# alphafox02/iridium-sniffer

Hardware: AMD Instinct MI355X
Metric: IQ Msamples/s end-to-end (detect->demod), 10 MHz cf32 (higher is better)
Workload: dtype f32

## Files before the change

iridium-sniffer_amd/csrc/scan_band.hip:

```cpp
#include <atomic>
#include <mutex>
#include "common.hpp"
#include "types.hpp"
#include "kernels.hpp"
#include "band_core.hpp"
#include "band_wave.hpp"

namespace irdm {

namespace {

__device__ __forceinline__ bool band_void(const BandParams &P, const BandWork &W)
{
    return __hip_atomic_load(W.bar + 5, __ATOMIC_RELAXED, __HIP_MEMORY_SCOPE_AGENT) == (unsigned)P.serial;
}

struct TlScope {
    unsigned long long *lo, *hi;
    __device__ __forceinline__ TlScope(const BandParams &P, const BandWork &W, int slot) : lo(nullptr), hi(nullptr)
    {
        if (P.tl_sel >= 0 && (threadIdx.x & 63) == 0 && slot >= 0 && slot < kBandTlSlots) {
            lo = W.tl + (size_t)P.tl_sel * 2 * kBandTlSlots + slot;
            hi = lo + kBandTlSlots;
            atomicMin(lo, (unsigned long long)wall_clock64());
// ... 49 lines not shown
    int bad = 0, ca = 0, cb = 0;
    for (int a = lane; a < na; a += 64) {
        if (A[a].cb < X - P.hw || A[a].cb >= X + P.hw) continue;
        ca++;
        bool found = false;
        for (int b = 0; b < nb && !found; b++) found = B[b].cb == A[a].cb && band_rec_same(A[a], B[b]);
        if (!found) bad = 1;
    }
    for (int b = lane; b < nb; b += 64)
        if (B[b].cb >= X - P.hw && B[b].cb < X + P.hw) cb++;
    for (int d = 32; d; d >>= 1) {
        ca += __shfl_xor(ca, d);
        cb += __shfl_xor(cb, d);
        bad |= __shfl_xor(bad, d);
    }
    return !(bad || ca != cb);
}

struct ZoneEnt {
    uint32_t cb, start_lo, idx;
};
constexpr int kZoneCap = 32;
constexpr size_t kZoneLdsBytes = 64 * kZoneCap * (sizeof(ZoneEnt) + sizeof(uint32_t)) + 128 * sizeof(uint32_t);

__device__ void boundaries_agree_lds(const BandParams &P, const BandWork &W, uint8_t *lds, int *s_fail, int nt)
{
    ZoneEnt *zb = reinterpret_cast<ZoneEnt *>(lds);
    uint32_t *za = reinterpret_cast<uint32_t *>(zb + 64 * kZoneCap);
    uint32_t *zc = za + 64 * kZoneCap;
    const int tid = threadIdx.x, gl = tid & 15;
    for (int t = tid; t < 128; t += nt) zc[t] = 0;
    __syncthreads();
    for (int i = tid >> 4; i + 1 < P.n_bands; i += nt >> 4) {
        const int X = (i + 1) * P.band_w;
        const BandRec *A = W.recs + (size_t)i * kBandRecCap, *B = W.recs + (size_t)(i + 1) * kBandRecCap;
        const int na = min((int)W.rec_count[i], kBandRecCap), nb = min((int)W.rec_count[i + 1], kBandRecCap);
        const int nmax = max(na, nb);
        for (int k = gl; k < nmax; k += 16) {
            const int cba = k < na ? A[k].cb : -0x40000000;
            const int cbb = k < nb ? B[k].cb : -0x40000000;
            const uint32_t stb = k < nb ? (uint32_t)B[k].start : 0u;
            if (cba >= X - P.hw && cba < X + P.hw) {
                const uint32_t at = atomicAdd(&zc[2 * i], 1u);
                if (at < (uint32_t)kZoneCap) za[i * kZoneCap + at] = (uint32_t)k;
            }
            if (cbb >= X - P.hw && cbb < X + P.hw) {
                const uint32_t at = atomicAdd(&zc[2 * i + 1], 1u);
                if (at < (uint32_t)kZoneCap) zb[i * kZoneCap + at] = ZoneEnt{ (uint32_t)cbb, stb, (uint32_t)k };
            }
        }
    }
    __syncthreads();
    int bad = 0;
    for (int i = tid >> 4; i + 1 < P.n_bands; i += nt >> 4) {
        const int X = (i + 1) * P.band_w;
        const BandRec *A = W.recs + (size_t)i * kBandRecCap, *B = W.recs + (size_t)(i + 1) * kBandRecCap;
        const int na = min((int)W.rec_count[i], kBandRecCap), nb = min((int)W.rec_count[i + 1], kBandRecCap);
        const int ca = (int)zc[2 * i], cb = (int)zc[2 * i + 1];
        if (ca != cb) {
            bad = 1;
        } else if (ca > kZoneCap) {
            for (int a = gl; a < na; a += 16) {
                if (A[a].cb < X - P.hw || A[a].cb >= X + P.hw) continue;
                bool found = false;
                for (int b = 0; b < nb && !found; b++) found = B[b].cb == A[a].cb && band_rec_same(A[a], B[b]);
                if (!found) bad = 1;
            }
        } else {
            for (int k = gl; k < ca; k += 16) {
                const BandRec ra = A[za[i * kZoneCap + k]];
                bool found = false;
                for (int j = 0; j < cb && !found; j++) {
                    const ZoneEnt e = zb[i * kZoneCap + j];
                    if (e.cb == (uint32_t)ra.cb && e.start_lo == (uint32_t)ra.start) found = band_rec_same(ra, B[e.idx]);
                }
                if (!found) bad = 1;
            }
        }
    }
    if (bad) atomicOr(s_fail, 1);
}

__device__ __forceinline__ SumStep make_step(const BandParams &P, int uf, int old, int slot)
{
    SumStep s;
    const uint32_t row = (uint32_t)P.n * 4u;
    s.nw_off = (uint32_t)uf * row;
    s.ol_off = (uint32_t)(old < 0 ? -old - 1 : old) * row;
    s.snap_off = slot >= 0 ? (uint32_t)slot * row : ~0u;
    s.pad = 0;
    return s;
}
__device__ __forceinline__ SumStep noop_step()
{
    SumStep s;
    s.nw_off = 0;
    s.ol_off = 0;
    s.snap_off = ~0u;
    s.pad = 0;
    return s;
}

struct PlanShared {
    int32_t part[kPlanThreads / 64 + 1];
    int mismatch, first, status, agree_fail;
    unsigned flags;
    int kstar;
};

constexpr int kPlanLdsFrames = 8192;
constexpr size_t kPlanLdsBytes = ((2 * kPlanLdsFrames + 2 + 15) & ~15) + sizeof(int32_t) * (2 * kPlanLdsFrames + 2);
static_assert(kZoneLdsBytes <= kPlanLdsBytes, "the boundary test's lists live in the plan's LDS before the plan needs it");

template <int NT>
__device__ void band_plan_body(const BandParams &P, const BandWork &W, const unsigned *__restrict__ counts,
                               DetState *__restrict__ st, int round, PlanShared &sh, uint8_t *lds,
                               const uint64_t *u_busy = nullptr, const uint64_t *u_forced = nullptr)
{
    const bool first = round == 0 || (P.spec_in && round == 1);
    if (!(P.spec_in && round == 1) || u_busy == nullptr) {
        u_busy = W.busy;
        u_forced = W.forced;
    }
    constexpr int kPlanThreads = NT;
    int32_t *s_part = sh.part;
    int &s_mismatch = sh.mismatch, &s_first = sh.first, &s_status = sh.status, &s_agree_fail = sh.agree_fail;
    unsigned &s_flags = sh.flags;
    const int tid = threadIdx.x;
    BandCtl *ctl = W.ctl;
    if (first) {
        if (tid == 0) {
            const unsigned prev = W.bar[4];
            s_status = (P.chained && prev != 1u) ? 1 : 0;
            if (s_status) __hip_atomic_store(W.bar + 5, (unsigned)P.serial, __ATOMIC_RELAXED, __HIP_MEMORY_SCOPE_AGENT);
            else W.bar[4] = 0;
        }
        __syncthreads();
        if (s_status) return;
        __syncthreads();
    } else if (band_void(P, W)) {
        return;
    }
    if (first) {
        if (tid < (int)(sizeof(BandCtl) / 4)) reinterpret_cast<uint32_t *>(ctl)[tid] = 0;
        if (tid == 0) {
            *W.flags = 0;
            st->n_gone = 0;
        }
        __syncthreads();
        if (round != 0 && tid == 0) ctl->h0 = st->hist_idx;
    }
    if (ctl->status != 0) return;
    const int F = P.n_frames;
    const uint64_t t_begin = wall_clock64();
    uint32_t *tp = ctl->tp + (round == 1 ? 0 : 8);
    auto stamp = [&](int i) {
        if (tid == 0 && round >= 1) tp[i] = (uint32_t)(wall_clock64() - t_begin);
    };

    if (tid == 0) {
        s_mismatch = 0;
        s_first = 0x7fffffff;
        s_flags = 0;
        s_status = 0;
        s_agree_fail = 0;
    }
    __syncthreads();
    if (round == 0) {
        int any = 0;
        for (int f = tid; f < F; f += kPlanThreads) {
            const unsigned c = counts[f];
            W.uq[f] = 0;
            W.uf[f] = 0;
            W.cnt_before[f] = 0;
            const int slot = c > 0 ? 0 : -1;
            W.slot_pre[f] = slot;
            W.slot_post[f] = slot;
            any |= c > 0 ? 1 : 0;
            if (c > (unsigned)P.list_cap) atomicOr(&s_flags, BAND_F_LIST);
        }
        if (any) atomicOr(&s_mismatch, 1);
        for (int i = tid; i < P.n_bands * P.occ_words; i += kPlanThreads) W.occ[i] = 0;
        for (int i = tid; i < P.occ_words; i += kPlanThreads) {
            W.busy[i] = 0;
            W.forced[i] = 0;
            W.conc[i] = 0;
        }
        for (int i = tid; i < P.n_bands; i += kPlanThreads) W.rec_count[i] = 0;
        for (int k = tid; k < 2 * kSumDepth + 1; k += kPlanThreads) W.steps[k] = noop_step();
        __syncthreads();
        if (tid == 0) {
            const int some = s_mismatch;
            ctl->h0 = st->hist_idx;
            W.need[0] = some;
            W.snap_slot[0] = some ? 0 : -1;
            ctl->n_upd = 0;
            ctl->n_snap = some;
            ctl->rounds = 1;
            if (s_flags) {
                ctl->flags = s_flags;
                ctl->status = 2;
            }
        }
        return;
    } else if (first) {
        for (int f = tid; f < F; f += kPlanThreads)
            if (counts[f] > (unsigned)P.list_cap) atomicOr(&s_flags, BAND_F_LIST);
        __syncthreads();
        if (s_flags) {
            if (tid == 0) {
                ctl->flags = s_flags;
                ctl->rounds = 1;
                ctl->status = 2;
            }
            return;
        }
        for (int f = tid; f < F; f += kPlanThreads) {
            W.uq[f] = ((u_busy[f >> 6] >> (f & 63)) & 1) ? 0 : 1;
            W.uf[f] = (uint8_t)((u_forced[f >> 6] >> (f & 63)) & 1);
        }
        if (P.selfcheck & 32) {
            __syncthreads();
            if (tid == 0 && F >= 8) W.uq[(3 * F) / 4] ^= 1;
            __syncthreads();
        }
    } else {
        for (int f = tid; f < F; f += kPlanThreads) {
            const int q = ((W.busy[f >> 6] >> (f & 63)) & 1) ? 0 : 1;
            const int fc = (int)((W.forced[f >> 6] >> (f & 63)) & 1);
            if (q != W.uq[f] || fc != W.uf[f]) {
                atomicAdd(&s_mismatch, 1);
                atomicMin(&s_first, f);
            }
        }
        for (int b = tid; b < P.occ_words; b += kPlanThreads)
            if (W.conc[b] >= (unsigned)P.max_bursts) atomicOr(&s_flags, BAND_F_SQUELCH);
        __syncthreads();
        stamp(0);
        if (P.selfcheck & 2) {
            for (int i = 1; i < P.n_bands; i++) {
                BandRec *B = W.recs + (size_t)i * kBandRecCap;
                const int X = i * P.band_w, nb = min((int)W.rec_count[i], kBandRecCap);
                for (int k = tid; k < nb; k += kPlanThreads)
                    if (B[k].cb >= X - P.hw && B[k].cb < X + P.hw) B[k].last_active += 1;
            }
            __syncthreads();
        }
        if (lds != nullptr) {
            boundaries_agree_lds(P, W, lds, &s_agree_fail, NT);
            if (P.selfcheck & 1) {
                __shared__ int s_other;
                if (tid == 0) s_other = 0;
                __syncthreads();
                for (int i = tid >> 6; i + 1 < P.n_bands; i += kPlanThreads / 64)
                    if (!boundary_agrees(P, W, i, tid & 63) && (tid & 63) == 0) atomicOr(&s_other, 1);
                __syncthreads();
                if (tid == 0 && s_other != s_agree_fail) atomicOr(&s_flags, BAND_F_CHECK);
            }
        } else {
            for (int i = tid >> 6; i + 1 < P.n_bands; i += kPlanThreads / 64)
                if (!boundary_agrees(P, W, i, tid & 63) && (tid & 63) == 0) atomicOr(&s_agree_fail, 1);
        }
        __syncthreads();
        stamp(1);
        if (tid == 0) {
            unsigned fl = s_flags | *W.flags;
            int status = 0;
            if (fl) {
                status = 2;
            } else if (s_mismatch == 0) {
                if (s_agree_fail) {
                    fl |= BAND_F_AGREE;
                    status = 2;
                } else {
                    status = 1;
                }
            } else if (round >= kBandRounds) {
                fl |= BAND_F_ITER;
                status = 2;
            }
            ctl->flags = fl;
            ctl->mismatch = s_mismatch;
            ctl->first_mismatch = s_first;
            ctl->rounds = round;
            ctl->status = status;
            s_status = status;
        }
        __syncthreads();
        if (s_status != 0) return;
        for (int f = tid; f < F; f += kPlanThreads) {
            W.uq[f] = ((W.busy[f >> 6] >> (f & 63)) & 1) ? 0 : 1;
            W.uf[f] = (uint8_t)((W.forced[f >> 6] >> (f & 63)) & 1);
        }
    }
    __syncthreads();
    if (round == 0 && s_flags) {
        if (tid == 0) {
            ctl->flags = s_flags;
            ctl->status = 2;
        }
        return;
    }

    if (lds != nullptr && F <= kPlanLdsFrames) {
        constexpr int FPT = kPlanLdsFrames / NT;
        uint8_t *s_need = lds;
        int32_t *s_slot = reinterpret_cast<int32_t *>(lds + ((2 * kPlanLdsFrames + 2 + 15) & ~15));
        const int f0 = tid * FPT;
        int uqb = 0, ufb = 0, cnz = 0, c_t = 0;
#pragma unroll
        for (int j = 0; j < FPT; j++) {
            const int f = f0 + j;
            if (f < F) {
                int q = ((u_busy[f >> 6] >> (f & 63)) & 1) ? 0 : 1;
                const int fc = (int)((u_forced[f >> 6] >> (f & 63)) & 1);
                if ((P.selfcheck & 32) && first && round == 1 && F >= 8 && f == (3 * F) / 4) q ^= 1;
                uqb |= q << j;
                ufb |= fc << j;
                cnz |= (counts[f] > 0 ? 1 : 0) << j;
                c_t += q + fc;
            }
        }
        __syncthreads();
        stamp(2);
        for (int i = tid; i < P.n_bands * P.occ_words; i += kPlanThreads) W.occ[i] = 0;
        for (int i = tid; i < P.occ_words; i += kPlanThreads) {
            W.busy[i] = 0;
            W.forced[i] = 0;
            W.conc[i] = 0;
        }
        for (int i = tid; i < P.n_bands; i += kPlanThreads) W.rec_count[i] = 0;
        const int lane = tid & 63, wave = tid >> 6;
        auto scan1 = [&](int v, int &total) {
            int incl = v;
            for (int d = 1; d < 64; d <<= 1) {
                const int o = __shfl_up(incl, d);
                if (lane >= d) incl += o;
            }
            if (lane == 63) s_part[wave] = incl;
            __syncthreads();
            int wb = 0, tot = 0;
            for (int w = 0; w < NT / 64; w++) {
                const int o = s_part[w];
                if (w < wave) wb += o;
                tot += o;
            }
            __syncthreads();
            total = tot;
            return wb + incl - v;
        };
        int n_upd = 0;
        const int base = scan1(c_t, n_upd);
        stamp(3);
        for (int k = tid; k <= n_upd + 1; k += kPlanThreads) s_need[k] = (P.sum_restart && k > 0 && (k & 63) == 0) ? 1 : 0;
        __syncthreads();
        {
            int k = base;
#pragma unroll
            for (int j = 0; j < FPT; j++) {
                const int f = f0 + j;
                if (f < F) {
                    const int q = (uqb >> j) & 1, fc = (ufb >> j) & 1;
                    if (f == s_first) sh.kstar = k;
                    if ((cnz >> j) & 1) {
                        s_need[k] = 1;
                        if (fc) s_need[k + 1] = 1;
                    }
                    if (fc) W.upd_frame[k++] = f;
                    if (q) W.upd_frame[k++] = f;
                }
            }
        }
        __syncthreads();
        stamp(4);
        const int kpt = (n_upd + 1 + NT - 1) / NT;
        const int k0 = tid * kpt, k1 = min(k0 + kpt, n_upd + 1);
        int nn = 0;
        for (int k = k0; k < k1; k++) nn += s_need[k];
        int n_snap = 0;
        int run = scan1(nn, n_snap);
        for (int k = k0; k < k1; k++) {
            const int nd = s_need[k];
            s_slot[k] = nd ? run : -1;
            run += nd;
        }
        if (tid == 0) W.snap_slot[0] = s_need[0] ? 0 : -1;
        __syncthreads();
        stamp(5);
        const int h0 = ctl->h0;
        for (int k = n_upd + tid; k < n_upd + 2 * kSumDepth + 1; k += kPlanThreads) W.steps[k] = noop_step();
        for (int k = tid; k < n_upd; k += kPlanThreads) {
            const int uf_k = W.upd_frame[k];
            const int old = k < kHistory ? -(((h0 + k) % kHistory) + 1) : W.upd_frame[k - kHistory];
            W.steps[k] = make_step(P, uf_k, old, s_slot[k + 1]);
        }
        {
            int k = base;
#pragma unroll
            for (int j = 0; j < FPT; j++) {
                const int f = f0 + j;
                if (f < F) {
                    const int q = (uqb >> j) & 1, fc = (ufb >> j) & 1, has = (cnz >> j) & 1;
                    const int pre = has ? s_slot[k] : -1;
                    W.slot_pre[f] = pre;
                    W.slot_post[f] = (has && fc) ? s_slot[k + 1] : pre;
                    k += q + fc;
                }
            }
        }
        __syncthreads();
        stamp(6);
        if (tid == 0) {
            ctl->n_upd = n_upd;
            ctl->n_snap = n_snap;
            ctl->rounds = round + 1;
            if (n_snap > W.snap_cap) {
                ctl->flags = BAND_F_SNAP;
                ctl->status = 2;
            }
            int kr = 0;
            if (P.sum_restart && !first && round >= 2 && s_first != 0x7fffffff && s_first < F) kr = (sh.kstar / 64) * 64;
            if (kr > n_upd) kr = (n_upd / 64) * 64;
            if (kr >= 64 && s_slot[kr] >= 0) {
                ctl->k_restart = kr;
                ctl->restart_slot = s_slot[kr];
                ctl->n_restarts++;
            } else {
                ctl->k_restart = 0;
                ctl->restart_slot = -1;
            }
        }
        return;
    }

    for (int i = tid; i < P.n_bands * P.occ_words; i += kPlanThreads) W.occ[i] = 0;
    for (int i = tid; i < P.occ_words; i += kPlanThreads) {
        W.busy[i] = 0;
        W.forced[i] = 0;
        W.conc[i] = 0;
    }
    for (int i = tid; i < P.n_bands; i += kPlanThreads) W.rec_count[i] = 0;

    for (int f = tid; f < F; f += kPlanThreads) W.tmp[f] = W.uq[f] + W.uf[f];
    __syncthreads();
    const int n_upd = block_scan<NT>(W.tmp, W.cnt_before, F, s_part);
    for (int k = tid; k <= n_upd; k += kPlanThreads) W.need[k] = 0;
    __syncthreads();
    for (int f = tid; f < F; f += kPlanThreads) {
        int k = W.cnt_before[f];
        if (counts[f] > 0) {
            W.need[k] = 1;
            if (W.uf[f]) W.need[k + 1] = 1;
        }
        if (W.uf[f]) W.upd_frame[k++] = f;
        if (W.uq[f]) W.upd_frame[k] = f;
    }
    __syncthreads();
    const int n_snap = block_scan<NT>(W.need, W.tmp, n_upd + 1, s_part);
    for (int k = tid; k <= n_upd; k += kPlanThreads) W.snap_slot[k] = W.need[k] ? W.tmp[k] : -1;
    __syncthreads();
    const int h0 = ctl->h0;
    for (int k = n_upd + tid; k < n_upd + 2 * kSumDepth + 1; k += kPlanThreads) W.steps[k] = noop_step();
    for (int k = tid; k < n_upd; k += kPlanThreads) {
        W.snap_after[k] = W.snap_slot[k + 1];
        W.old_row[k] = k < kHistory ? -(((h0 + k) % kHistory) + 1) : W.upd_frame[k - kHistory];
        W.steps[k] = make_step(P, W.upd_frame[k], W.old_row[k], W.snap_after[k]);
    }
    for (int f = tid; f < F; f += kPlanThreads) {
        const int k = W.cnt_before[f];
        const int pre = counts[f] > 0 ? W.snap_slot[k] : -1;
        W.slot_pre[f] = pre;
        W.slot_post[f] = (counts[f] > 0 && W.uf[f]) ? W.snap_slot[k + 1] : pre;
    }
    if (tid == 0) {
        ctl->n_upd = n_upd;
        ctl->n_snap = n_snap;
// ... 110 lines not shown
        const bool more = k0 + 2 * kSumDepth < n;
        const uint4 dnn = steps4[k0 + 4 * kSumDepth + lane];
        IRDM_SUM_LOAD(nwB, olB, d, 1, k0 + kSumDepth)
        IRDM_SUM_CONSUME(nwA, olA, d, 0, k0)
        if (more) { IRDM_SUM_LOAD(nwA, olA, dn, 0, k0 + 2 * kSumDepth) }
        IRDM_SUM_CONSUME(nwB, olB, d, 1, k0 + kSumDepth)
        d = dn;
        dn = dnn;
    }
#undef IRDM_SUM_LOAD
#undef IRDM_SUM_CONSUME
#undef IRDM_SUM_STEP
    W.sum_new[b] = s;
    smin_out[b] = smin;
    if (!(pre[b] <= 0.9f * P.thr * smin)) atomicOr(W.flags, BAND_F_STALE);
}

__global__ __launch_bounds__(64) void band_sum_kernel(BandParams P, BandWork W, const float *__restrict__ mag,
                                                      const float *__restrict__ hist, const float *__restrict__ sum,
                                                      const float *__restrict__ pre, float *__restrict__ smin_out,
                                                      const SumStep *__restrict__ steps, float *__restrict__ snap)
{
    IRDM_DETECTOR_PRIO();
    TlScope tl(P, W, 4 * (W.ctl->rounds - 1) + 1);
    if (band_void(P, W) || W.ctl->status != 0) return;
    band_sum_body(P, W, mag, hist, sum, pre, smin_out, steps, snap, (int)blockIdx.x * 64 + (int)threadIdx.x);
}

constexpr int kWalkWaveGroups = 256;

template <int NW>
__global__ __launch_bounds__(256) void band_walk_wave_kernel(BandParams P, BandWork W, BandIO io, const DetState *__restrict__ st)
{
    IRDM_DETECTOR_PRIO();
    TlScope tl(P, W, 4 * (W.ctl->rounds - 1) + 3);
    if (band_void(P, W) || W.ctl->status != 0) return;
    io.act_in = st->act;
    io.n_act_in = (int32_t)wv_first((uint32_t)st->n_act);
    const int lane = threadIdx.x & 63;
    const int gw = (int)wv_first((uint32_t)(blockIdx.x * 4 + (threadIdx.x >> 6))), n_waves = (int)gridDim.x * 4;
    const int n_pairs = P.n_bands * P.occ_words;
    unsigned long long *tl_stat = nullptr;
    if (P.tl_sel >= 0)
        tl_stat = W.tl + (size_t)P.tl_sel * 2 * kBandTlSlots + kBandTlSlots + (W.ctl->rounds - 1 == 0 ? 26 : 28);
    int wave_events = 0;
    const unsigned long long t_wave = tl_stat ? wall_clock64() : 0;
    for (int p0 = gw; p0 < n_pairs; p0 += 64 * n_waves) {
        const int pl = p0 + lane * n_waves;
        bool work = false;
        if (pl < n_pairs) {
            const int band = pl / P.occ_words, blk = pl % P.occ_words;
            work = blk == 0 || band_segment_starts(io.occ + (size_t)band * P.occ_words, blk, P.gap, false) != 0;
        }
        uint64_t todo = __builtin_amdgcn_ballot_w64(work);
        while (todo) {
            const int j = __builtin_ctzll(todo);
            todo &= todo - 1;
            const int p = p0 + j * n_waves;
            const int band = p / P.occ_words, blk = p % P.occ_words;
            bool carried = false;
            int events = 0;
            if (blk == 0) {
                WaveWalker<NW> w(P, io, band, lane);
                if (w.load_carried() > 0) {
                    carried = true;
                    w.run(0, true);
                    events += w.n_events;
                }
            }
            uint64_t starts = wv_first64(band_segment_starts(io.occ + (size_t)band * P.occ_words, blk, P.gap, carried));
            while (starts) {
                const int q = __builtin_ctzll(starts);
                starts &= starts - 1;
                WaveWalker<NW> w(P, io, band, lane);
                w.run(64 * blk + q, false);
                events += w.n_events;
            }
            wave_events += events;
            if (tl_stat && lane == 0) {
                atomicMax(tl_stat, (unsigned long long)events);
                atomicAdd(tl_stat + 1, (unsigned long long)events);
            }
        }
    }
    if (tl_stat && lane == 0 && W.ctl->rounds - 1 != 0) {
        unsigned long long *x = W.tl + (size_t)P.tl_sel * 2 * kBandTlSlots + kBandTlSlots + 30;
        atomicMax(x, (unsigned long long)wave_events);
        atomicMax(x + 1, wall_clock64() - t_wave);
    }
}

__device__ __forceinline__ void band_cross_wave(const BandParams &P, const BandWork &W, unsigned c,
                                                const ListEntry *__restrict__ entries, int f, uint32_t *s_bits, int lane)
{
    const int N = P.n;
    for (int w = lane; w < N / 32; w += 64) s_bits[w] = 0;
    __builtin_amdgcn_fence(__ATOMIC_RELEASE, "wavefront");
    __builtin_amdgcn_wave_barrier();
    const float *srow = W.snap + (size_t)W.slot_pre[f] * N;
    const ListEntry *e = entries + (size_t)f * P.list_cap;
    float *rq = W.relq + (size_t)f * N;
    for (unsigned i = lane; i < c; i += 64) {
        const int bin = e[i].bin;
        const float base = srow[bin];
        const float rel = base > 0 ? e[i].mag / base : 0.0f;
        if (rel > P.thr) {
            atomicOr(&s_bits[bin >> 5], 1u << (bin & 31));
            rq[bin] = rel;
        }
    }
    __builtin_amdgcn_fence(__ATOMIC_ACQ_REL, "wavefront");
    __builtin_amdgcn_wave_barrier();
    uint32_t *out = reinterpret_cast<uint32_t *>(W.cross) + (size_t)f * (N / 32);
    for (int w = lane; w < N / 32; w += 64) out[w] = s_bits[w];
    if (lane < P.n_bands) {
        const int w0 = (lane * P.band_w - P.band_w / 2) / 32, nw = 2 * P.band_w / 32;
        uint32_t any = 0;
        for (int k = 0; k < nw; k++) {
            const int w = w0 + k;
            if (w >= 0 && w < N / 32) any |= s_bits[w];
        }
        if (any) atomicOr(reinterpret_cast<unsigned long long *>(&W.occ[(size_t)lane * P.occ_words + (f >> 6)]), 1ull << (f & 63));
    }
    __builtin_amdgcn_fence(__ATOMIC_ACQ_REL, "wavefront");
    __builtin_amdgcn_wave_barrier();
}

constexpr int kCrossGroups = 256;

__global__ __launch_bounds__(256) void band_cross_w_kernel(BandParams P, BandWork W, const unsigned *__restrict__ counts,
                                                           const ListEntry *__restrict__ entries)
{
    IRDM_DETECTOR_PRIO();
    TlScope tl(P, W, 4 * (W.ctl->rounds - 1) + 2);
    __shared__ uint32_t s_bits_all[4][16384 / 32];
    if (band_void(P, W) || W.ctl->status != 0) return;
    const int lane = threadIdx.x & 63, wave = threadIdx.x >> 6;
    const int gw = (int)blockIdx.x * 4 + wave, n_waves = (int)gridDim.x * 4;
    uint32_t *s_bits = s_bits_all[wave];
    for (int f0 = gw; f0 < P.n_frames; f0 += 64 * n_waves) {
        const int fl = f0 + lane * n_waves;
        const unsigned cl = fl < P.n_frames ? counts[fl] : 0u;
        uint64_t todo = __builtin_amdgcn_ballot_w64(cl != 0 && cl <= (unsigned)P.list_cap);
        while (todo) {
            const int j = __builtin_ctzll(todo);
            todo &= todo - 1;
            const unsigned c = (unsigned)__builtin_amdgcn_readlane((int)cl, j);
            band_cross_wave(P, W, c, entries, f0 + j * n_waves, s_bits, lane);
        }
    }
}


__global__ __launch_bounds__(256) void band_spec_prep_kernel(BandParams P, BandWork S, const unsigned *__restrict__ counts,
                                                              const float *__restrict__ sum_src, DetState *__restrict__ st_spec,
                                                              int have_prev)
{
    IRDM_DETECTOR_PRIO();
    const int tid = threadIdx.x, F = P.n_frames;
    __shared__ unsigned s_n;
    if (tid == 0) s_n = 0;
    __syncthreads();
    if (have_prev)
        for (int band = tid >> 4; band < P.n_bands; band += 256 / 16) {
            const int cnt = min((int)S.rec_count[band], kBandRecCap);
            for (int j = tid & 15; j < cnt; j += 16) {
                const BandRec &r = S.recs[(size_t)band * kBandRecCap + j];
                if (!(r.flags & 1) || r.stop >= 0) continue;
                const unsigned at = atomicAdd(&s_n, 1u);
                if (at < (unsigned)kMaxActive) {
                    ActiveBurst a;
                    a.id = 0; a.start = (uint64_t)r.start; a.last_active = (uint64_t)r.last_active;
                    a.center_bin = r.cb; a.peak_rel = r.rel; a.base_sum = r.base; a.pad = 0;
                    st_spec->act[at] = a;
                }
            }
        }
    __syncthreads();
    if (tid == 0) st_spec->n_act = (uint32_t)min(s_n, (unsigned)kMaxActive);
    if (tid < (int)(sizeof(BandCtl) / 4)) reinterpret_cast<uint32_t *>(S.ctl)[tid] = 0;
    for (int f = tid; f < F; f += 256) {
        const int slot = counts[f] > 0 ? 0 : -1;
        S.slot_pre[f] = slot;
        S.slot_post[f] = slot;
    }
    for (int i = tid; i < P.n_bands * P.occ_words; i += 256) S.occ[i] = 0;
    for (int i = tid; i < P.occ_words; i += 256) {
        S.busy[i] = 0;
        S.forced[i] = 0;
        S.conc[i] = 0;
    }
    for (int i = tid; i < P.n_bands; i += 256) S.rec_count[i] = 0;
    for (int b = tid; b < P.n; b += 256) S.snap[b] = sum_src[b];
    __syncthreads();
    if (tid == 0) {
        *S.flags = 0;
        S.ctl->rounds = 1;
        S.snap_slot[0] = 0;
    }
}

__device__ void lds_bitonic_sort(uint64_t *key, uint16_t *val, int np)
{
    for (int k = 2; k <= np; k <<= 1) {
        for (int j = k >> 1; j > 0; j >>= 1) {
            for (int i = threadIdx.x; i < np / 2; i += blockDim.x) {
                const int lo = ((i & ~(j - 1)) << 1) | (i & (j - 1)), hi = lo | j;
                const uint64_t a = key[lo], b = key[hi];
                if ((a > b) == ((lo & k) == 0)) {
                    key[lo] = b;
                    key[hi] = a;
                    const uint16_t va = val[lo];
                    val[lo] = val[hi];
                    val[hi] = va;
                }
            }
            __syncthreads();
        }
    }
}

__device__ void band_commit_body(const BandParams &P, const BandWork &W, DetState *__restrict__ st,
                                 float *__restrict__ sum, GoneBurst *__restrict__ gone, int gone_cap,
                                 unsigned char *smem_raw)
{
    const int kPlanThreads = (int)blockDim.x;
    uint64_t *s_key = reinterpret_cast<uint64_t *>(smem_raw);
    uint16_t *s_val = reinterpret_cast<uint16_t *>(s_key + kBandMaxTotal);
    uint32_t *rank_of = W.rank;
    __shared__ unsigned s_n, s_carried, s_gone;
    BandCtl *ctl = W.ctl;
    if (band_void(P, W) || ctl->status != 1 || ctl->committed) return;
    const int tid = threadIdx.x;
    if (tid == 0) {
        s_n = 0;
        s_carried = 0;
        s_gone = 0;
    }
    __syncthreads();
    for (int band = tid >> 4; band < P.n_bands; band += kPlanThreads / 16) {
        {
            const int cnt = min((int)W.rec_count[band], kBandRecCap);
            for (int j = tid & 15; j < cnt; j += 16) {
                const int i = band * kBandRecCap + j;
                const BandRec &r = W.recs[i];
                if (!(r.flags & 1)) continue;
                const unsigned at = atomicAdd(&s_n, 1u);
                if (at < (unsigned)kBandMaxTotal) W.tot[at] = i;
                if (r.cf < 0) atomicAdd(&s_carried, 1u);
                if (r.stop >= 0) atomicAdd(&s_gone, 1u);
            }
        }
    }
    __syncthreads();
    const int n = (int)s_n, n_carried = (int)s_carried, n_gone = (int)s_gone;
    if (n > kBandMaxTotal || n_gone > gone_cap) {
        if (tid == 0) {
            ctl->flags |= n > kBandMaxTotal ? BAND_F_TOTAL : BAND_F_GONECAP;
            ctl->n_gone = n_gone;
            ctl->status = 2;
        }
        return;
    }
    for (int t = tid; t < n; t += kPlanThreads) {
        const BandRec &r = W.recs[W.tot[t]];
        uint64_t key;
        if (r.cf < 0) {
            key = (uint64_t)r.seq;
        } else {
            uint32_t rb;
            __builtin_memcpy(&rb, &r.rel, 4);
            key = (1ull << 63) | ((uint64_t)r.cf << 46) | ((uint64_t)(0xffffffffu - rb) << 14) | (uint64_t)r.cb;
        }
        s_key[t] = key;
        s_val[t] = (uint16_t)t;
    }
    int np = 2;
    while (np < n) np <<= 1;
    for (int t = n + tid; t < np; t += kPlanThreads) {
        s_key[t] = ~0ull;
        s_val[t] = 0xffff;
    }
    __syncthreads();
    lds_bitonic_sort(s_key, s_val, np);
    for (int q = tid; q < n; q += kPlanThreads) rank_of[s_val[q]] = (uint32_t)q;
    __syncthreads();
    const uint64_t id0 = st->burst_id;
    for (int t = tid; t < n; t += kPlanThreads) {
        const BandRec &r = W.recs[W.tot[t]];
        W.ids[t] = r.cf < 0 ? st->act[r.seq].id : id0 + 10ull * (uint64_t)((int)rank_of[t] - n_carried);
    }
    for (int t = tid; t < n; t += kPlanThreads) {
        const BandRec &r = W.recs[W.tot[t]];
        s_key[t] = r.stop >= 0 ? (((uint64_t)((r.stop - (int64_t)P.idx0) >> P.log_n)) << 32) | rank_of[t]
                               : (1ull << 63) | rank_of[t];
        s_val[t] = (uint16_t)t;
    }
    for (int t = n + tid; t < np; t += kPlanThreads) {
        s_key[t] = ~0ull;
        s_val[t] = 0xffff;
    }
    __syncthreads();
    lds_bitonic_sort(s_key, s_val, np);
    for (int pos = tid; pos < n; pos += kPlanThreads) {
        const int t = s_val[pos];
        const BandRec &r = W.recs[W.tot[t]];
        const uint64_t id = W.ids[t];
        if (r.stop >= 0) {
            GoneBurst g;
            g.id = id; g.start = (uint64_t)r.start; g.stop = (uint64_t)r.stop; g.last_active = (uint64_t)r.last_active;
            g.center_bin = r.cb; g.peak_rel = r.rel; g.base_sum = r.base; g.pad = 0;
            gone[pos] = g;
        } else {
            ActiveBurst a;
            a.id = id; a.start = (uint64_t)r.start; a.last_active = (uint64_t)r.last_active;
            a.center_bin = r.cb; a.peak_rel = r.rel; a.base_sum = r.base; a.pad = 0;
            st->act[pos - n_gone] = a;
        }
    }
    for (int b = tid; b < P.n; b += kPlanThreads) sum[b] = W.sum_new[b];
    if (tid == 0) {
        const int F = P.n_frames;
        st->index += (uint64_t)F * (uint64_t)P.n;
        st->burst_id = id0 + 10ull * (uint64_t)(n - n_carried);
        st->hist_idx = (ctl->h0 + ctl->n_upd) % kHistory;
        st->squelch = st->squelch > F ? st->squelch - F : 0;
        st->n_act = n - n_gone;
        st->n_gone = (uint32_t)n_gone;
        ctl->n_gone = n_gone;
        ctl->n_total = n;
        ctl->committed = 1;
        W.bar[4] = 1;
    }
}

__global__ __launch_bounds__(kPlanThreads) void band_commit_kernel(BandParams P, BandWork W, DetState *__restrict__ st,
                                                                   float *__restrict__ sum, GoneBurst *__restrict__ gone,
                                                                   int gone_cap)
{
    IRDM_DETECTOR_PRIO();
    TlScope tl(P, W, 24);
    extern __shared__ __attribute__((aligned(16))) unsigned char smem_raw[];
    band_commit_body(P, W, st, sum, gone, gone_cap, smem_raw);
}

constexpr int kExportBlocks = 32;

__global__ __launch_bounds__(256) void band_history_kernel(BandParams P, BandWork W, const float *__restrict__ mag,
                                                           float *__restrict__ hist, const DetState *__restrict__ st,
                                                           const uint32_t *__restrict__ gone, int gone_cap,
                                                           uint32_t *__restrict__ hp_gone, uint32_t *__restrict__ hp_hdr,
                                                           uint32_t *__restrict__ hp_ctl)
{
    IRDM_DETECTOR_PRIO();
    TlScope tl(P, W, 25);
    const BandCtl *ctl = W.ctl;
    if (band_void(P, W)) {
        if (hp_ctl && blockIdx.x == 0 && threadIdx.x == 0) {
            __hip_atomic_store(hp_ctl + 2, (uint32_t)BAND_F_CHAIN, __ATOMIC_RELAXED, __HIP_MEMORY_SCOPE_SYSTEM);
            __hip_atomic_store(hp_ctl + 0, 2u, __ATOMIC_RELAXED, __HIP_MEMORY_SCOPE_SYSTEM);
            __threadfence_system();
        }
        return;
    }
    if (hp_hdr && blockIdx.x < kExportBlocks)
        gone_export_body(st, gone, gone_cap, hp_gone, hp_hdr, reinterpret_cast<const uint32_t *>(ctl), hp_ctl,
                         (int)(sizeof(BandCtl) / 4), kExportBlocks);
    if (ctl->status != 1 || !ctl->committed) return;
    const int k = ctl->n_upd - 1 - (int)blockIdx.x;
    if (k < 0) return;
    const float4 *src = reinterpret_cast<const float4 *>(mag + (size_t)W.upd_frame[k] * P.n);
    float4 *dst = reinterpret_cast<float4 *>(hist + (size_t)((ctl->h0 + k) % kHistory) * P.n);
    for (int i0 = threadIdx.x; i0 < P.n / 4; i0 += 8 * 256) {
        float4 v[8];
#pragma unroll
        for (int u = 0; u < 8; u++)
            if (i0 + 256 * u < P.n / 4) v[u] = src[i0 + 256 * u];
#pragma unroll
        for (int u = 0; u < 8; u++)
            if (i0 + 256 * u < P.n / 4) dst[i0 + 256 * u] = v[u];
    }
}

}

int band_list_cap(int n) { return n < kBandListCap ? n : kBandListCap; }

int band_scan_supported(const DetParams &D, BandParams *out, int n_frames, uint64_t idx0)
{
    BandParams P;
    P.n = D.n;
    P.log_n = 31 - __builtin_clz((unsigned)(D.n > 0 ? D.n : 1));
    P.nw64 = D.n / 64;
    P.n_frames = n_frames;
    P.occ_words = (n_frames + 63) / 64;
    P.hw = D.width / 2;
    P.pre_len = D.pre_len;
    P.post_len = D.post_len;
    P.max_len = D.max_len;
    P.max_bursts = D.max_bursts;
    P.band_w = P.hw <= 20 ? 128 : 256;
    P.n_bands = D.n / P.band_w;
    P.gap = (D.post_len + D.n - 1) / D.n;
    P.thr = D.threshold;
    P.idx0 = idx0;
    P.list_cap = band_list_cap(D.n);
    if (out) *out = P;
    if (D.n < 2048 || D.n > 16384 || D.n != (1 << P.log_n) || P.n_bands < 1 || P.n_bands > 64) return 0;
    if (P.hw < 1 || 2 * P.hw + 8 > P.band_w / 2) return 0;
    if (P.gap < 1 || P.gap >= 64) return 0;
    if (D.max_bursts <= 0 || D.max_bursts > kMaxActive - 64) return 0;
    return 1;
}

size_t band_work_bytes(int n, size_t max_chunk, bool spec)
{
    const size_t F = max_chunk / (size_t)n + 2;
    size_t b = 0;
    auto add = [&](size_t x) { b += (x + 255) & ~(size_t)255; };
    add(sizeof(BandCtl));
    add(F); add(F);
    add(4 * (F + 2)); add(4 * (2 * F + 4));
    add(4 * (2 * F + 4)); add(4 * (2 * F + 4)); add(4 * (2 * F + 4));
    add(sizeof(SumStep) * (2 * F + 4 + 3 * kSumDepth + 6 * kSumDepth));
    add(4 * (2 * F + 4)); add(4 * (2 * F + 4));
    add(4 * F); add(4 * F);
    add(F * (size_t)n / 8);
    add(F * (size_t)n * 4);
    add((spec ? 2 : F + 2 + F / 32 + 4) * (size_t)n * 4);
    add(64 * ((F + 63) / 64) * 8);
    add(((F + 63) / 64) * 8); add(((F + 63) / 64) * 8); add(((F + 63) / 64) * 4);
    add(sizeof(BandRec) * 64 * kBandRecCap); add(4 * 64);
    add(4 * (size_t)n); add(4 * kBandMaxTotal); add(8 * kBandMaxTotal); add(256);
    add(256); add(4 * kBandMaxTotal);
    add(8 * 4 * kBandTlSlots);
    return b;
}

int band_work_carve(BandWork *W, void *base, int n, size_t max_chunk, bool spec)
{
    const size_t F = max_chunk / (size_t)n + 2;
    unsigned char *p = static_cast<unsigned char *>(base);
    auto take = [&](size_t x) { void *q = p; p += (x + 255) & ~(size_t)255; return q; };
    W->ctl = static_cast<BandCtl *>(take(sizeof(BandCtl)));
    W->uq = static_cast<uint8_t *>(take(F));
    W->uf = static_cast<uint8_t *>(take(F));
    W->cnt_before = static_cast<int32_t *>(take(4 * (F + 2)));
    W->tmp = static_cast<int32_t *>(take(4 * (2 * F + 4)));
    W->upd_frame = static_cast<int32_t *>(take(4 * (2 * F + 4)));
    W->old_row = static_cast<int32_t *>(take(4 * (2 * F + 4)));
    W->snap_after = static_cast<int32_t *>(take(4 * (2 * F + 4)));
    W->steps = static_cast<SumStep *>(take(sizeof(SumStep) * (2 * F + 4 + 3 * kSumDepth + 6 * kSumDepth)));
    W->need = static_cast<int32_t *>(take(4 * (2 * F + 4)));
    W->snap_slot = static_cast<int32_t *>(take(4 * (2 * F + 4)));
    W->slot_pre = static_cast<int32_t *>(take(4 * F));
    W->slot_post = static_cast<int32_t *>(take(4 * F));
    W->cross = static_cast<uint64_t *>(take(F * (size_t)n / 8));
    W->relq = static_cast<float *>(take(F * (size_t)n * 4));
    W->snap = static_cast<float *>(take((spec ? 2 : F + 2 + F / 32 + 4) * (size_t)n * 4));
    W->snap_cap = (int)(spec ? 2 : F + 2 + F / 32 + 4);
    W->occ = static_cast<uint64_t *>(take(64 * ((F + 63) / 64) * 8));
    W->busy = static_cast<uint64_t *>(take(((F + 63) / 64) * 8));
    W->forced = static_cast<uint64_t *>(take(((F + 63) / 64) * 8));
    W->conc = static_cast<uint32_t *>(take(((F + 63) / 64) * 4));
    W->recs = static_cast<BandRec *>(take(sizeof(BandRec) * 64 * kBandRecCap));
    W->rec_count = static_cast<uint32_t *>(take(4 * 64));
    W->sum_new = static_cast<float *>(take(4 * (size_t)n));
    W->tot = static_cast<uint32_t *>(take(4 * kBandMaxTotal));
    W->ids = static_cast<uint64_t *>(take(8 * kBandMaxTotal));
    W->flags = static_cast<uint32_t *>(take(256));
    W->bar = static_cast<unsigned *>(take(256));
    W->rank = static_cast<uint32_t *>(take(4 * kBandMaxTotal));
    W->tl = static_cast<unsigned long long *>(take(8 * 4 * kBandTlSlots));
    return 0;
}

static unsigned next_launch_serial()
{
    static std::atomic<unsigned> launch_serial{ 0 };
    unsigned serial = launch_serial.fetch_add(1) + 1;
    if (serial == 0) serial = launch_serial.fetch_add(1) + 1;
    return serial;
}

int launch_band_spec(const DetParams &D, BandWork S, DetState *st_spec, const float *sum_src, int n_frames, uint64_t idx0,
                     const unsigned *counts, const ListEntry *entries, int have_prev, hipStream_t stream, const BandTune &tune)
{
    BandParams P;
    if (!band_scan_supported(D, &P, n_frames, idx0) || n_frames < 1) return -1;
    P.serial = (int32_t)next_launch_serial();
    P.selfcheck = tune.selfcheck & 8;
    BandIO io;
    io.cross = S.cross;
    io.occ = S.occ;
    io.relq = S.relq;
    io.snap = S.snap;
    io.slot_post = S.slot_post;
    io.act_in = nullptr;
    io.n_act_in = 0;
    io.recs = S.recs;
    io.rec_count = S.rec_count;
    io.busy = S.busy;
    io.forced = S.forced;
    io.conc = S.conc;
    io.flags = S.flags;
    hipLaunchKernelGGL(band_spec_prep_kernel, dim3(1), dim3(256), 0, stream, P, S, counts, sum_src, st_spec, have_prev);
    hipLaunchKernelGGL(band_cross_w_kernel, dim3(kCrossGroups), dim3(256), 0, stream, P, S, counts, entries);
    if (P.band_w == 128)
        hipLaunchKernelGGL((band_walk_wave_kernel<4>), dim3(kWalkWaveGroups), dim3(256), 0, stream, P, S, io, st_spec);
    else
        hipLaunchKernelGGL((band_walk_wave_kernel<8>), dim3(kWalkWaveGroups), dim3(256), 0, stream, P, S, io, st_spec);
    return hipGetLastError() == hipSuccess ? 0 : -1;
}

int launch_band_scan(const DetParams &D, BandWork W, DetState *st, float *sum, float *hist, const float *mag,
                     int n_frames, uint64_t idx0, const unsigned *counts, const ListEntry *entries, const float *pre,
                     float *smin, GoneBurst *gone, int gone_cap, int round_begin, int round_end, GoneBurst *hp_gone,
                     uint32_t *hp_hdr, void *hp_ctl, int hp_cap, int chained, int tl_sel, hipStream_t stream,
                     const BandTune &tune, const uint32_t *gate_flag, uint32_t gate_seq, uint32_t *gate_err, const void *gate_src,
                     size_t gate_bytes, const BandWork *spec, hipEvent_t sums_done)
{
    if (spec && round_begin != 1) return -1;
    const uint64_t *ub = spec ? spec->busy : nullptr, *uf = spec ? spec->forced : nullptr;
    bool sums_noted = sums_done == nullptr;
    BandParams P;
    if (!band_scan_supported(D, &P, n_frames, idx0) || n_frames < 1) return -1;
    P.serial = (int32_t)next_launch_serial();
    P.chained = chained;
    P.spec_in = spec ? 1 : 0;
    P.sum_restart = tune.sum_restart;
    P.selfcheck = tune.selfcheck;
    P.tl_sel = tune.timeline && tl_sel >= 0 && tl_sel < 2 ? tl_sel : -1;
    if (P.tl_sel >= 0 && (round_begin == 0 || spec)) {
        unsigned long long *half = W.tl + (size_t)P.tl_sel * 2 * kBandTlSlots;
        (void)hipMemsetAsync(half, 0xff, 8 * kBandTlSlots, stream);
        (void)hipMemsetAsync(half + kBandTlSlots, 0, 8 * kBandTlSlots, stream);
    }
    BandIO io;
    io.cross = W.cross;
    io.occ = W.occ;
    io.relq = W.relq;
    io.snap = W.snap;
    io.slot_post = W.slot_post;
    io.act_in = nullptr;
    io.n_act_in = 0;
    io.recs = W.recs;
    io.rec_count = W.rec_count;
    io.busy = W.busy;
    io.forced = W.forced;
    io.conc = W.conc;
    io.flags = W.flags;
    const size_t commit_lds = (size_t)kBandMaxTotal * (8 + 2);
    (void)hipFuncSetAttribute((const void *)band_commit_kernel, hipFuncAttributeMaxDynamicSharedMemorySize, (int)commit_lds);
    (void)hipFuncSetAttribute((const void *)band_plan_kernel<kPlanThreads>, hipFuncAttributeMaxDynamicSharedMemorySize, (int)kPlanLdsBytes);
    for (int round = round_begin; round <= round_end; round++) {
        if (round > round_begin || round_begin == 0 || spec) {
            const size_t plan_lds = (P.selfcheck & 16) ? 0 : kPlanLdsBytes;
            const float *pre0 = round == 0 ? pre : nullptr;
            hipLaunchKernelGGL(band_plan_kernel<kPlanThreads>, dim3(1), dim3(kPlanThreads), plan_lds, stream, P, W, counts, st, round, sum,
                               gone, gone_cap, pre0, smin, ub, uf);
        }
        if (round == round_end) break;
        if (gate_flag && round == (round_begin > 1 ? round_begin : 1)) {
            if (launch_wait_host_flag(gate_flag, gate_seq, gate_err, stream) != 0) return -1;
            if (hipMemcpyAsync(hist, gate_src, gate_bytes, hipMemcpyDeviceToDevice, stream) != hipSuccess) return -1;
        }
        if (round >= 1)
            hipLaunchKernelGGL(band_sum_kernel, dim3(P.n / 64), dim3(64), 0, stream, P, W, mag, hist, sum, pre, smin, W.steps, W.snap);
        if (!sums_noted && round >= 1) {
            if (hipEventRecord(sums_done, stream) != hipSuccess) return -1;
            sums_noted = true;
        }
        hipLaunchKernelGGL(band_cross_w_kernel, dim3(kCrossGroups), dim3(256), 0, stream, P, W, counts, entries);
        if (P.band_w == 128)
            hipLaunchKernelGGL((band_walk_wave_kernel<4>), dim3(kWalkWaveGroups), dim3(256), 0, stream, P, W, io, st);
        else
            hipLaunchKernelGGL((band_walk_wave_kernel<8>), dim3(kWalkWaveGroups), dim3(256), 0, stream, P, W, io, st);
    }
    if (P.selfcheck & 16)
        hipLaunchKernelGGL(band_commit_kernel, dim3(1), dim3(kPlanThreads), commit_lds, stream, P, W, st, sum, gone, gone_cap);
    static_assert(kHistory >= kExportBlocks, "the export rides on the history pass's first workgroups");
    hipLaunchKernelGGL(band_history_kernel, dim3(kHistory), dim3(256), 0, stream, P, W, mag, hist, st,
                       reinterpret_cast<const uint32_t *>(gone), hp_cap < gone_cap ? hp_cap : gone_cap,
                       reinterpret_cast<uint32_t *>(hp_gone), hp_hdr, static_cast<uint32_t *>(hp_ctl));
    return hipGetLastError() == hipSuccess ? 0 : -1;
}

}
```

Before: 76170.

## Parallelize spec prep across blocks and pack plan-kernel bitmap checks per thread

The speculative prep kernel now runs on many blocks, batches its counts/snap copies, and gathers active records with a prefix-sum over band counts instead of a nested per-band loop. In the plan kernel's LDS path, the uq/uf mismatch check and update use one byte of the busy/forced bitmaps and one 8-byte word per thread, and the first-round list-cap check is folded into the existing per-frame pass. The sum copy-back is batched 16-wide, and timeline slots are added for the spec kernels. This aims to cut serial single-block work and redundant global passes, at the cost of more complex indexing and assumptions about alignment and bitmap byte layout.

Measured after the change: 77600 (median of 5 runs). 1.02x the previous value.

```diff
diff --git a/iridium-sniffer_amd/csrc/scan_band.hip b/iridium-sniffer_amd/csrc/scan_band.hip
--- a/iridium-sniffer_amd/csrc/scan_band.hip
+++ b/iridium-sniffer_amd/csrc/scan_band.hip
@@ -225,6 +225,7 @@
     }
     if (ctl->status != 0) return;
     const int F = P.n_frames;
+    const bool lds_path = lds != nullptr && F <= kPlanLdsFrames;
     const uint64_t t_begin = wall_clock64();
     uint32_t *tp = ctl->tp + (round == 1 ? 0 : 8);
     auto stamp = [&](int i) {
@@ -276,6 +277,7 @@
             }
         }
         return;
+    } else if (first && lds_path) {
     } else if (first) {
         for (int f = tid; f < F; f += kPlanThreads)
             if (counts[f] > (unsigned)P.list_cap) atomicOr(&s_flags, BAND_F_LIST);
@@ -298,12 +300,33 @@
             __syncthreads();
         }
     } else {
-        for (int f = tid; f < F; f += kPlanThreads) {
-            const int q = ((W.busy[f >> 6] >> (f & 63)) & 1) ? 0 : 1;
-            const int fc = (int)((W.forced[f >> 6] >> (f & 63)) & 1);
-            if (q != W.uq[f] || fc != W.uf[f]) {
-                atomicAdd(&s_mismatch, 1);
-                atomicMin(&s_first, f);
+        if (lds_path) {
+            const int f0 = tid * (kPlanLdsFrames / NT);
+            static_assert(kPlanLdsFrames / NT == 8, "a thread's frames are one byte of the bitmaps and one 8-byte word of uq / uf");
+            if (f0 < F) {
+                const unsigned bb = reinterpret_cast<const uint8_t *>(W.busy)[tid], fb = reinterpret_cast<const uint8_t *>(W.forced)[tid];
+                const uint64_t pq = *reinterpret_cast<const uint64_t *>(W.uq + f0), pf = *reinterpret_cast<const uint64_t *>(W.uf + f0);
+                unsigned qbits = 0, fbits = 0;
+#pragma unroll
+                for (int j = 0; j < 8; j++) {
+                    qbits |= (unsigned)((pq >> (8 * j)) & 1) << j;
+                    fbits |= (unsigned)((pf >> (8 * j)) & 1) << j;
+                }
+                const unsigned valid = F - f0 >= 8 ? 0xffu : (1u << (F - f0)) - 1u;
+                const unsigned bad = (((~bb & 0xffu) ^ qbits) | (fb ^ fbits)) & valid;
+                if (bad) {
+                    atomicAdd(&s_mismatch, __popc(bad));
+                    atomicMin(&s_first, f0 + __ffs((int)bad) - 1);
+                }
+            }
+        } else {
+            for (int f = tid; f < F; f += kPlanThreads) {
+                const int q = ((W.busy[f >> 6] >> (f & 63)) & 1) ? 0 : 1;
+                const int fc = (int)((W.forced[f >> 6] >> (f & 63)) & 1);
+                if (q != W.uq[f] || fc != W.uf[f]) {
+                    atomicAdd(&s_mismatch, 1);
+                    atomicMin(&s_first, f);
+                }
             }
         }
         for (int b = tid; b < P.occ_words; b += kPlanThreads)
@@ -361,10 +384,11 @@
         }
         __syncthreads();
         if (s_status != 0) return;
-        for (int f = tid; f < F; f += kPlanThreads) {
-            W.uq[f] = ((W.busy[f >> 6] >> (f & 63)) & 1) ? 0 : 1;
-            W.uf[f] = (uint8_t)((W.forced[f >> 6] >> (f & 63)) & 1);
-        }
+        if (!lds_path)
+            for (int f = tid; f < F; f += kPlanThreads) {
+                W.uq[f] = ((W.busy[f >> 6] >> (f & 63)) & 1) ? 0 : 1;
+                W.uf[f] = (uint8_t)((W.forced[f >> 6] >> (f & 63)) & 1);
+            }
     }
     __syncthreads();
     if (round == 0 && s_flags) {
@@ -375,7 +399,7 @@
         return;
     }
 
-    if (lds != nullptr && F <= kPlanLdsFrames) {
+    if (lds_path) {
         constexpr int FPT = kPlanLdsFrames / NT;
         uint8_t *s_need = lds;
         int32_t *s_slot = reinterpret_cast<int32_t *>(lds + ((2 * kPlanLdsFrames + 2 + 15) & ~15));
@@ -390,11 +414,32 @@
                 if ((P.selfcheck & 32) && first && round == 1 && F >= 8 && f == (3 * F) / 4) q ^= 1;
                 uqb |= q << j;
                 ufb |= fc << j;
-                cnz |= (counts[f] > 0 ? 1 : 0) << j;
+                const unsigned c = counts[f];
+                cnz |= (c > 0 ? 1 : 0) << j;
                 c_t += q + fc;
-            }
-        }
-        __syncthreads();
+                if (first && c > (unsigned)P.list_cap) atomicOr(&s_flags, BAND_F_LIST);
+            }
+        }
+        __syncthreads();
+        if (first && s_flags) {
+            if (tid == 0) {
+                ctl->flags = s_flags;
+                ctl->rounds = 1;
+                ctl->status = 2;
+            }
+            return;
+        }
+        static_assert(FPT == 8, "a thread's frames are one 8-byte word of uq / uf");
+        if (f0 < F) {
+            uint64_t wq = 0, wf = 0;
+#pragma unroll
+            for (int j = 0; j < FPT; j++) {
+                wq |= (uint64_t)((uqb >> j) & 1) << (8 * j);
+                wf |= (uint64_t)((ufb >> j) & 1) << (8 * j);
+            }
+            *reinterpret_cast<uint64_t *>(W.uq + f0) = wq;
+            *reinterpret_cast<uint64_t *>(W.uf + f0) = wf;
+        }
         stamp(2);
         for (int i = tid; i < P.n_bands * P.occ_words; i += kPlanThreads) W.occ[i] = 0;
         for (int i = tid; i < P.occ_words; i += kPlanThreads) {
@@ -811,48 +856,100 @@
 }
 
 
+constexpr int kSpecPrepGroups = 64;
+constexpr int kSpecPrepBatch = 4;
+
+inline int spec_prep_groups(const BandParams &P)
+{
+    int widest = P.n_frames > P.n ? P.n_frames : P.n;
+    if (P.n_bands * P.occ_words > widest) widest = P.n_bands * P.occ_words;
+    const int groups = (widest + 255) / 256;
+    return groups < kSpecPrepGroups ? groups : kSpecPrepGroups;
+}
+
 __global__ __launch_bounds__(256) void band_spec_prep_kernel(BandParams P, BandWork S, const unsigned *__restrict__ counts,
                                                               const float *__restrict__ sum_src, DetState *__restrict__ st_spec,
                                                               int have_prev)
 {
     IRDM_DETECTOR_PRIO();
+    TlScope tl(P, S, 0);
     const int tid = threadIdx.x, F = P.n_frames;
-    __shared__ unsigned s_n;
-    if (tid == 0) s_n = 0;
-    __syncthreads();
-    if (have_prev)
-        for (int band = tid >> 4; band < P.n_bands; band += 256 / 16) {
-            const int cnt = min((int)S.rec_count[band], kBandRecCap);
-            for (int j = tid & 15; j < cnt; j += 16) {
-                const BandRec &r = S.recs[(size_t)band * kBandRecCap + j];
-                if (!(r.flags & 1) || r.stop >= 0) continue;
-                const unsigned at = atomicAdd(&s_n, 1u);
-                if (at < (unsigned)kMaxActive) {
-                    ActiveBurst a;
-                    a.id = 0; a.start = (uint64_t)r.start; a.last_active = (uint64_t)r.last_active;
-                    a.center_bin = r.cb; a.peak_rel = r.rel; a.base_sum = r.base; a.pad = 0;
-                    st_spec->act[at] = a;
-                }
-            }
-        }
-    __syncthreads();
-    if (tid == 0) st_spec->n_act = (uint32_t)min(s_n, (unsigned)kMaxActive);
-    if (tid < (int)(sizeof(BandCtl) / 4)) reinterpret_cast<uint32_t *>(S.ctl)[tid] = 0;
-    for (int f = tid; f < F; f += 256) {
-        const int slot = counts[f] > 0 ? 0 : -1;
-        S.slot_pre[f] = slot;
-        S.slot_post[f] = slot;
-    }
-    for (int i = tid; i < P.n_bands * P.occ_words; i += 256) S.occ[i] = 0;
-    for (int i = tid; i < P.occ_words; i += 256) {
+    const int gt = (int)blockIdx.x * 256 + tid, gn = (int)gridDim.x * 256;
+    for (int f0 = gt; f0 < F; f0 += kSpecPrepBatch * gn) {
+        unsigned c[kSpecPrepBatch];
+#pragma unroll
+        for (int u = 0; u < kSpecPrepBatch; u++)
+            if (f0 + u * gn < F) c[u] = counts[f0 + u * gn];
+#pragma unroll
+        for (int u = 0; u < kSpecPrepBatch; u++)
+            if (f0 + u * gn < F) {
+                const int slot = c[u] > 0 ? 0 : -1;
+                S.slot_pre[f0 + u * gn] = slot;
+                S.slot_post[f0 + u * gn] = slot;
+            }
+    }
+    for (int b0 = gt; b0 < P.n; b0 += kSpecPrepBatch * gn) {
+        float v[kSpecPrepBatch];
+#pragma unroll
+        for (int u = 0; u < kSpecPrepBatch; u++)
+            if (b0 + u * gn < P.n) v[u] = sum_src[b0 + u * gn];
+#pragma unroll
+        for (int u = 0; u < kSpecPrepBatch; u++)
+            if (b0 + u * gn < P.n) S.snap[b0 + u * gn] = v[u];
+    }
+    for (int i = gt; i < P.n_bands * P.occ_words; i += gn) S.occ[i] = 0;
+    for (int i = gt; i < P.occ_words; i += gn) {
         S.busy[i] = 0;
         S.forced[i] = 0;
         S.conc[i] = 0;
     }
-    for (int i = tid; i < P.n_bands; i += 256) S.rec_count[i] = 0;
-    for (int b = tid; b < P.n; b += 256) S.snap[b] = sum_src[b];
+    if (blockIdx.x != 0) return;
+
+    __shared__ unsigned s_n;
+    __shared__ int s_off[65];
+    if (tid == 0) s_n = 0;
+    {
+        const int lane = tid & 63;
+        int incl = (have_prev && lane < P.n_bands) ? min((int)S.rec_count[lane], kBandRecCap) : 0;
+        for (int d = 1; d < 64; d <<= 1) {
+            const int o = __shfl_up(incl, d);
+            if (lane >= d) incl += o;
+        }
+        if (tid < 64) s_off[tid + 1] = incl;
+        if (tid == 0) s_off[0] = 0;
+    }
+    __syncthreads();
+    if (tid < P.n_bands) S.rec_count[tid] = 0;
+    const int total = s_off[64];
+    for (int t0 = tid; t0 < total; t0 += kSpecPrepBatch * 256) {
+        BandRec r[kSpecPrepBatch];
+#pragma unroll
+        for (int u = 0; u < kSpecPrepBatch; u++) {
+            const int t = t0 + u * 256;
+            if (t < total) {
+                int band = 0;
+#pragma unroll
+                for (int step = 32; step; step >>= 1)
+                    if (s_off[band + step] <= t) band += step;
+                r[u] = S.recs[(size_t)band * kBandRecCap + (t - s_off[band])];
+            }
+        }
+#pragma unroll
+        for (int u = 0; u < kSpecPrepBatch; u++) {
+            if (t0 + u * 256 >= total || !(r[u].flags & 1) || r[u].stop >= 0) continue;
+            const unsigned at = atomicAdd(&s_n, 1u);
+            if (at < (unsigned)kMaxActive) {
+                ActiveBurst a;
+                a.id = 0; a.start = (uint64_t)r[u].start; a.last_active = (uint64_t)r[u].last_active;
+                a.center_bin = r[u].cb; a.peak_rel = r[u].rel; a.base_sum = r[u].base; a.pad = 0;
+                st_spec->act[at] = a;
+            }
+        }
+    }
+    if (tid < (int)(sizeof(BandCtl) / 4)) reinterpret_cast<uint32_t *>(S.ctl)[tid] = 0;
     __syncthreads();
     if (tid == 0) {
+        st_spec->n_act = (uint32_t)min(s_n, (unsigned)kMaxActive);
         *S.flags = 0;
         S.ctl->rounds = 1;
         S.snap_slot[0] = 0;
@@ -977,7 +1074,15 @@
             st->act[pos - n_gone] = a;
         }
     }
-    for (int b = tid; b < P.n; b += kPlanThreads) sum[b] = W.sum_new[b];
+    for (int b0 = tid; b0 < P.n; b0 += 16 * kPlanThreads) {
+        float v[16];
+#pragma unroll
+        for (int u = 0; u < 16; u++)
+            if (b0 + u * kPlanThreads < P.n) v[u] = W.sum_new[b0 + u * kPlanThreads];
+#pragma unroll
+        for (int u = 0; u < 16; u++)
+            if (b0 + u * kPlanThreads < P.n) sum[b0 + u * kPlanThreads] = v[u];
+    }
     if (tid == 0) {
         const int F = P.n_frames;
         st->index += (uint64_t)F * (uint64_t)P.n;
@@ -1149,6 +1254,11 @@
     if (!band_scan_supported(D, &P, n_frames, idx0) || n_frames < 1) return -1;
     P.serial = (int32_t)next_launch_serial();
     P.selfcheck = tune.selfcheck & 8;
+    P.tl_sel = tune.timeline ? 0 : -1;
+    if (P.tl_sel >= 0) {
+        (void)hipMemsetAsync(S.tl, 0xff, 8 * kBandTlSlots, stream);
+        (void)hipMemsetAsync(S.tl + kBandTlSlots, 0, 8 * kBandTlSlots, stream);
+    }
     BandIO io;
     io.cross = S.cross;
     io.occ = S.occ;
@@ -1163,7 +1273,7 @@
     io.forced = S.forced;
     io.conc = S.conc;
     io.flags = S.flags;
-    hipLaunchKernelGGL(band_spec_prep_kernel, dim3(1), dim3(256), 0, stream, P, S, counts, sum_src, st_spec, have_prev);
+    hipLaunchKernelGGL(band_spec_prep_kernel, dim3(spec_prep_groups(P)), dim3(256), 0, stream, P, S, counts, sum_src, st_spec, have_prev);
     hipLaunchKernelGGL(band_cross_w_kernel, dim3(kCrossGroups), dim3(256), 0, stream, P, S, counts, entries);
     if (P.band_w == 128)
         hipLaunchKernelGGL((band_walk_wave_kernel<4>), dim3(kWalkWaveGroups), dim3(256), 0, stream, P, S, io, st_spec);
@@ -1194,6 +1304,10 @@
         unsigned long long *half = W.tl + (size_t)P.tl_sel * 2 * kBandTlSlots;
         (void)hipMemsetAsync(half, 0xff, 8 * kBandTlSlots, stream);
         (void)hipMemsetAsync(half + kBandTlSlots, 0, 8 * kBandTlSlots, stream);
+        if (spec) {
+            (void)hipMemcpyAsync(half, spec->tl, 8 * 4, hipMemcpyDeviceToDevice, stream);
+            (void)hipMemcpyAsync(half + kBandTlSlots, spec->tl + kBandTlSlots, 8 * 4, hipMemcpyDeviceToDevice, stream);
+        }
     }
     BandIO io;
     io.cross = W.cross;
```
